# talmolab/VNL-Brax-Imitation

Measured on AMD Instinct MI355X. Metric: env-steps/sec (whole node), rodent imitation, num_envs=4096/GPU, higher is better.
Workload: dtype f32; 1 GPU; rodent imitation rollout, single groom clip, 4096 envs/GPU: intention-policy forward (HIP) -> RodentTracking.step (5 substeps, CG 6/6) -> auto-reset on -> Transition logging (unroll 20, the 20 steps replayed as one captured hipGraph); envs_per_gpu=4096, clips=1, parallelism=env-sharded x1, no data-path collective

## Files before the change

__graft_entry__.py:

```python
from __future__ import annotations

import os
import sys

ROOT = os.path.dirname(os.path.abspath(__file__))
if ROOT not in sys.path:
    sys.path.insert(0, ROOT)


def build() -> None:
    import vnl_brax_imitation_amd
    from vnl_brax_imitation_amd.csrc import build as hip_build

    from concurrent.futures import ThreadPoolExecutor

    with ThreadPoolExecutor(9) as pool:
        futs = {v: pool.submit(hip_build.build, variant=v)
                for v in ("product", "spill", "noblk", "nospec", "tail", "plain", "vmemplain", "ldsplain", "sgprplain")}
        paths = {v: f.result() for v, f in futs.items()}
    path = paths["product"]
    assert all(os.path.exists(p_) for p_ in paths.values()), paths
    from oracle import oracle as _oracle

    _oracle.build()
    from vnl_brax_imitation_amd import _lib

    _lib.load_library(path)
    print(f"[build] {path} ok; oracle ok")


def smoke() -> None:
    import numpy as np
    import torch

    sys.path.insert(0, os.path.join(ROOT, "tests"))
    import helpers as H
    from vnl_brax_imitation_amd.envs.rodent import RodentTracking

    assert torch.cuda.is_available(), "smoke() needs a HIP device"
    B = 256
    env = RodentTracking(H.reference_clip(), num_envs=B, device="cuda:0", **H.env_kwargs())
    rng = np.random.default_rng(0)
    sf = rng.integers(0, 235, B).astype(np.int32)
    noise = (1e-3 * rng.standard_normal((B, 74))).astype(np.float32)
    st = env.reset(start_frame=torch.from_numpy(sf), noise=torch.from_numpy(noise))
    act = np.clip(0.3 * rng.standard_normal((B, 30)), -1, 1).astype(np.float32)
    o = H.make_oracle(env, "f64")
    ost = o.env_reset(sf, noise)
    e_reset = H.scaled_err(st.pipeline_state.qacc_warmstart.cpu().numpy(), ost["qacc_warmstart"])
    e_obs = H.scaled_err(st.obs.cpu().numpy(), ost["obs"])
    import parity as P
# ... 33 lines not shown
```

vnl-brax-imitation_amd/csrc/build.py:

```python
from __future__ import annotations

import os
import subprocess
import sys

HERE = os.path.dirname(os.path.abspath(__file__))
SOURCES = ["vnl_lib.hip", "vnl_policy.hip", "vnl_ppo.hip", "vnl_domain.hip"]
DEPS = SOURCES + ["vnl_env_kernels.h", "vnl_body.h", "vnl_types.h", "vnl_philox.h", "vnl_policy_train.h", "../../include/vnl.h"]
OUT = os.path.join(HERE, "libvnl.so")

VARIANTS = {
    "product": ("libvnl.so", ["-DVNL_KERNEL_ATTR=__attribute__((amdgpu_waves_per_eu(2,2)))"]),
    "prof": ("libvnl_prof.so", ["-DVNL_PROFILE", "-DVNL_KERNEL_ATTR=__attribute__((amdgpu_waves_per_eu(2,2)))"]),
    "knobs": ("libvnl_knobs.so", ["-DVNL_STAGE_KNOBS", "-DVNL_KERNEL_ATTR=__attribute__((amdgpu_waves_per_eu(2,2)))"]),
    "spill": ("libvnl_spill.so", ["-DVNL_KERNEL_ATTR=__attribute__((amdgpu_waves_per_eu(4,4)))"]),
    "noblk": ("libvnl_noblk.so", ["-DVNL_NO_BLK", "-DVNL_KERNEL_ATTR=__attribute__((amdgpu_waves_per_eu(2,2)))"]),
    "tail": ("libvnl_tail.so", ["-DVNL_SOLVER_TAIL", "-DVNL_KERNEL_ATTR=__attribute__((amdgpu_waves_per_eu(2,2)))"]),
    "plain": ("libvnl_plain.so", ["-DVNL_SOLVER_PLAIN", "-DVNL_KERNEL_ATTR=__attribute__((amdgpu_waves_per_eu(2,2)))"]),
    "vmemplain": ("libvnl_vmemplain.so", ["-DVNL_VMEM_PLAIN", "-DVNL_KERNEL_ATTR=__attribute__((amdgpu_waves_per_eu(2,2)))"]),
    "ldsplain": ("libvnl_ldsplain.so", ["-DVNL_LDS_PLAIN", "-DVNL_KERNEL_ATTR=__attribute__((amdgpu_waves_per_eu(2,2)))"]),
    "sgprplain": ("libvnl_sgprplain.so", ["-DVNL_SGPR_PLAIN", "-DVNL_KERNEL_ATTR=__attribute__((amdgpu_waves_per_eu(2,2)))"]),
    "nospec": ("libvnl_nospec.so", ["-DVNL_NO_SPEC", "-DVNL_KERNEL_ATTR=__attribute__((amdgpu_waves_per_eu(2,2)))"]),
}
ENV_KERNELS = ("vnl_step_kernel", "vnl_reset_kernel", "vnl_reset_done_kernel")


def resource_usage(stderr_text: str) -> dict:
    out, name = {}, None
    for line in stderr_text.splitlines():
        if "Function Name:" in line:
            name = line.split("Function Name:")[1].split()[0]
            out[name] = {}
        elif name and "remark:" in line:
            body = line.split("remark:")[1].split("[-Rpass")[0].strip()
            key, _, val = body.rpartition(":")
            try:
                out[name][key.strip()] = int(val.strip())
            except ValueError:
                pass
    return out


def build(force: bool = False, verbose: bool = False, profile: bool = False, knobs: bool = False,
          variant: str | None = None) -> str:
    variant = variant or ("prof" if profile else ("knobs" if knobs else "product"))
    fname, defs = VARIANTS[variant]
    out = os.path.join(HERE, fname)
    deps = [os.path.join(HERE, d) for d in DEPS] + [os.path.abspath(__file__)]
    newest = max(os.path.getmtime(d) for d in deps)
    if not force and os.path.exists(out) and os.path.getmtime(out) >= newest:
        return out
    hipcc = os.environ.get("HIPCC", "/opt/rocm/bin/hipcc")
    objdir = os.path.join(HERE, "_obj", variant)
    os.makedirs(objdir, exist_ok=True)
# ... 68 lines not shown
```

vnl-brax-imitation_amd/csrc/vnl_body.h:

```cpp
#pragma once
#include <math.h>
#ifdef VNL_FORKJOIN_DEFINED
#include <assert.h>
#endif

#include "vnl_types.h"

#ifndef VNL_HD
#define VNL_HD __device__ __forceinline__
#endif
#include "vnl_philox.h"

#ifndef VNL_FORKJOIN_DEFINED
#define VNL_LANES 64
#define VNL_ROWS_PER_LANE 8
#define VNL_ROWS_SMALL 5
#define VNL_CHAIN_WIDTH 8
#define VNL_ROWSETS_1 1
#define VNL_ROWSETS_2 2
#define VNL_FOR(i, n) for (int i = (int)lane; i < (n); i += VNL_LANES)
#define VNL_SERIAL if (lane == 0)
#define VNL_SYNC() __builtin_amdgcn_fence(__ATOMIC_ACQ_REL, "wavefront")
#define VNL_SYNC_GLOBAL()                                     \
  do {                                                        \
    __builtin_amdgcn_fence(__ATOMIC_ACQ_REL, "wavefront");    \
    asm volatile("s_waitcnt vmcnt(0)" ::: "memory");          \
    __builtin_amdgcn_fence(__ATOMIC_ACQ_REL, "wavefront");    \
  } while (0)
#define VNL_LDS_DECL(name) extern __shared__ __align__(16) vreal name[]
VNL_HD float vnl_wave_sum(float x) {
#define VNL_DPP_STEP(ctrl) x += __builtin_bit_cast(float, __builtin_amdgcn_update_dpp(0, __builtin_bit_cast(int, x), ctrl, 0xf, 0xf, true))
  VNL_DPP_STEP(0xB1);
  VNL_DPP_STEP(0x4E);
  VNL_DPP_STEP(0x141);
  VNL_DPP_STEP(0x140);
#undef VNL_DPP_STEP
  x += __builtin_bit_cast(float, __builtin_amdgcn_update_dpp(0, __builtin_bit_cast(int, x), 0x142, 0xa, 0xf, false));
  x += __builtin_bit_cast(float, __builtin_amdgcn_update_dpp(0, __builtin_bit_cast(int, x), 0x143, 0xc, 0xf, false));
  return __builtin_bit_cast(float, __builtin_amdgcn_readlane(__builtin_bit_cast(int, x), 63));
}
VNL_HD float vnl_wave_sum16(float x) {
#define VNL_DPP_STEP(ctrl) x += __builtin_bit_cast(float, __builtin_amdgcn_update_dpp(0, __builtin_bit_cast(int, x), ctrl, 0xf, 0xf, true))
  VNL_DPP_STEP(0xB1);
  VNL_DPP_STEP(0x4E);
  VNL_DPP_STEP(0x141);
  VNL_DPP_STEP(0x140);
#undef VNL_DPP_STEP
  return __builtin_bit_cast(float, __builtin_amdgcn_readlane(__builtin_bit_cast(int, x), 0));
}
VNL_HD bool vnl_wave_any(bool x) { return __ballot(x) != 0ull; }
VNL_HD float vnl_wave_scan(float x) {
#define VNL_DPP_SCAN(ctrl, rmask) \
  x += __builtin_bit_cast(float, __builtin_amdgcn_update_dpp(0, __builtin_bit_cast(int, x), ctrl, rmask, 0xf, false))
  VNL_DPP_SCAN(0x111, 0xf);
  VNL_DPP_SCAN(0x112, 0xf);
  VNL_DPP_SCAN(0x114, 0xf);
  VNL_DPP_SCAN(0x118, 0xf);
  VNL_DPP_SCAN(0x142, 0xa);
  VNL_DPP_SCAN(0x143, 0xc);
#undef VNL_DPP_SCAN
  return x;
}
#define VNL_SCAN_ADD(x, run) (x = vnl_wave_scan(x))
#define VNL_WAVE_ITEMS(n) VNL_LANES
#define VNL_PAD_ITEMS(n) (((n) + VNL_LANES - 1) / VNL_LANES * VNL_LANES)
#define VNL_SCAN_ADD_C(x, run, carry) \
  (x = vnl_wave_scan(x) + carry, carry = __builtin_bit_cast(float, __builtin_amdgcn_readlane(__builtin_bit_cast(int, x), 63)))
#define VNL_PERLANE(T, name) T name
#define VNL_AT(name, j) name
#define VNL_GETF(name, a) __builtin_bit_cast(float, __builtin_amdgcn_readlane(__builtin_bit_cast(int, name), a))
#define VNL_GETI(name, a) __builtin_amdgcn_readlane(name, a)
#define VNL_ROWGETI(name, q, l) __builtin_amdgcn_readlane(name[q], l)
#define VNL_ROWGETF(expr, q, l) __builtin_bit_cast(float, __builtin_amdgcn_readlane(__builtin_bit_cast(int, expr), l))
VNL_HD float vnl_seg_sum(float x, unsigned cont, int steps) {
#define VNL_DPP_SEG(ctrl, bit)                                                                                          \
  do {                                                                                                                  \
    const float t_ = __builtin_bit_cast(float, __builtin_amdgcn_update_dpp(0, __builtin_bit_cast(int, x), ctrl, 0xf, 0xf, true)); \
    x += (cont & (bit)) ? t_ : 0.0f;                                                                                     \
  } while (0)
  if (steps > 0) VNL_DPP_SEG(0x101, 1u);
  if (steps > 1) VNL_DPP_SEG(0x102, 2u);
  if (steps > 2) VNL_DPP_SEG(0x104, 4u);
  if (steps > 3) VNL_DPP_SEG(0x108, 8u);
#undef VNL_DPP_SEG
  return x;
}
#define VNL_SEG_SUM(part, dsc, steps) (part = vnl_seg_sum(part, (dsc) >> 28, steps))
#define VNL_WAVE_FENCE() __builtin_amdgcn_fence(__ATOMIC_ACQ_REL, "wavefront")
#define VNL_LINE_HEADERS(out, base, stride)                                                       \
  do {                                                                                            \
    int hv_ = (int)(base)[((int)lane < VNL_FAC_LINES ? (int)lane : VNL_FAC_LINES - 1) * (stride)]; \
    _Pragma("unroll") for (int k_ = 0; k_ < VNL_FAC_LINES; k_++) out[k_] = __builtin_amdgcn_readlane(hv_, k_); \
  } while (0)
#define VNL_COUNT(pred) __popcll(__ballot(pred))
#define VNL_RANK(pred, run, rank)                                                   \
  do {                                                                              \
    const unsigned long long b_ = __ballot(pred);                                   \
    rank = run + (int)__popcll(b_ & ((1ull << (threadIdx.x & 63)) - 1ull));         \
    run += (int)__popcll(b_);                                                       \
  } while (0)
#define VNL_UNIFORM_I(x) __builtin_amdgcn_readfirstlane(x)
VNL_HD float vnl_recip(float x) {
  float r = __builtin_amdgcn_rcpf(x);
  return r * (2.0f - x * r);
}
#endif

#ifndef VNL_FORKJOIN_DEFINED
VNL_HD void vnl_count_add(uint32_t* p) { atomicAdd(p, 1u); }
VNL_HD int vnl_cdf_cell(const uint32_t* cdf, int ncell, uint32_t x, unsigned lane) {
  int lo = 0, len = ncell - 1;
  while (len > VNL_LANES) {
    const int stride = (len + VNL_LANES - 1) / VNL_LANES, end = lo + len;
    const int p = lo + ((int)lane + 1) * stride - 1;
    const bool le = p < end && cdf[p] <= x;
    const int k = (int)__popcll(__ballot(le));
    lo = lo + k * stride < end ? lo + k * stride : end;
    len = end - lo < stride - 1 ? end - lo : stride - 1;
  }
  const bool le = (int)lane < len && cdf[lo + (int)lane] <= x;
  return lo + (int)__popcll(__ballot(le));
}
#else
VNL_HD void vnl_count_add(uint32_t* p) { *p += 1u; }
VNL_HD int vnl_cdf_cell(const uint32_t* cdf, int ncell, uint32_t x, unsigned) {
  int lo = 0, hi = ncell - 1;
  while (lo < hi) {
    const int mid = (lo + hi) >> 1;
    if (cdf[mid] <= x) lo = mid + 1; else hi = mid;
  }
  return lo;
}
#endif

#ifdef VNL_PROFILE
#define VNL_NPROF 40
__device__ unsigned long long g_vnl_prof[VNL_NPROF];
#define VNL_PROF(i)                                                                             \
// ... 429 lines not shown
  }

  VNL_HD void body_inertias(bool with_com) const {
    V3 O = ref_point();
    V3 csum = v3(vreal(0.), vreal(0.), vreal(0.));
    VNL_FOR(b, MI(nbody)) {
      int o = LO(P) + 10 * b;
      if (b == 0) {
        for (int k = 0; k < 10; k++) s[o + k] = vreal(0.);
        continue;
      }
      const int ob = m.body_out[b];
      M3 R = qmat(gquat4(ob));
      vreal mass = par_row<P_MASS>()[b];
      V3 xip = gpos3(ob) + mmul(R, t3(par_row<P_IPOS>(), b));
      csum = csum + xip * mass;
      V3 r = xip - O;
      const vreal* I6 = par_row<P_INERTIA6>() + 6 * b;
      vreal Ib[9] = {I6[0], I6[3], I6[4], I6[3], I6[1], I6[5], I6[4], I6[5], I6[2]};
      vreal T[9];
      for (int i = 0; i < 3; i++)
        for (int k = 0; k < 3; k++)
          T[3 * i + k] = R.a[3 * i] * Ib[k] + R.a[3 * i + 1] * Ib[3 + k] + R.a[3 * i + 2] * Ib[6 + k];
      vreal rr = dot(r, r);
      s[o + 0] = T[0] * R.a[0] + T[1] * R.a[1] + T[2] * R.a[2] + mass * (rr - r.x * r.x);
      s[o + 1] = T[3] * R.a[3] + T[4] * R.a[4] + T[5] * R.a[5] + mass * (rr - r.y * r.y);
      s[o + 2] = T[6] * R.a[6] + T[7] * R.a[7] + T[8] * R.a[8] + mass * (rr - r.z * r.z);
      s[o + 3] = T[0] * R.a[3] + T[1] * R.a[4] + T[2] * R.a[5] - mass * r.x * r.y;
      s[o + 4] = T[0] * R.a[6] + T[1] * R.a[7] + T[2] * R.a[8] - mass * r.x * r.z;
      s[o + 5] = T[3] * R.a[6] + T[4] * R.a[7] + T[5] * R.a[8] - mass * r.y * r.z;
      s[o + 6] = r.x * mass, s[o + 7] = r.y * mass, s[o + 8] = r.z * mass, s[o + 9] = mass;
    }
    if (with_com) {
      vreal cx = vnl_wave_sum(csum.x), cy = vnl_wave_sum(csum.y), cz = vnl_wave_sum(csum.z);
      VNL_SERIAL { st3(LO(com), v3(cx * total_mass_inv(), cy * total_mass_inv(), cz * total_mass_inv())); }
    }
    VNL_SYNC();
  }

  VNL_HD void tree_accumulate(int base, int width) const {
    VNL_FOR(k, width) {
      vreal carry = vreal(0.);
      int b = MI(nbody) - 1;
      constexpr int G = 8;
      for (; b >= 1 && (b & (G - 1)) != G - 1; b--) {
        const int o = base + width * b + k;
        const vreal v = s[o] + carry;
        const int p = parent_of(b);
        if (carry != vreal(0.)) s[o] = v;
        if (p == b - 1) {
          carry = v;
        } else {
          carry = vreal(0.);
          if (p > 0) s[base + width * p + k] += v;
        }
      }
      for (; b >= G - 1; b -= G) {
        const int b0 = b - (G - 1);
        const int o = base + width * b0 + k;
        unsigned pw[G / 4];
#pragma unroll
        for (int j = 0; j < G / 4; j++) pw[j] = (unsigned)VNL_UNIFORM_I((int)((const unsigned*)(s + LO(tab_body)))[(b0 >> 2) + j]);
        vreal x[G], x0[G];
#pragma unroll
        for (int j = 0; j < G; j++) x0[j] = x[j] = s[o + width * j];
#pragma unroll
        for (int j = G - 1; j >= 0; j--) {
// ... 910 lines not shown
    int X0 = LO(P) + 10 * MI(nbody);
    dof_prefix(LO(qvel), LO(LD));
    const int cv = cvel_at();
    VNL_FOR(b, MI(nbody)) st6(cv + 6 * b, path_sum(LO(LD), m.body_pathseg + 8 * b));
    VNL_SYNC();
    VNL_PROF(2);
    int ca = X0;
    const int QB = LO(LD) + 6 * (MI(nv) + 1);
    S6 run = S6{v3(0, 0, 0), v3(0, 0, 0)}, carry = run;
    VNL_FOR(b, VNL_PAD_ITEMS(MI(nbody))) {
      S6 acc = S6{v3(0, 0, 0), v3(0, 0, 0)};
      if (b > 0 && b < MI(nbody)) {
        S6 vel = ld6(cv + 6 * parent_of(b));
        int jn = m.body_jntnum[b], ja = m.body_jntadr[b];
        for (int k = 0; k < jn; k++) {
          int j = ja + k, da = m.jnt_dofadr[j];
          if (m.jnt_type[j] == VNL_JNT_FREE) {
            for (int t = 0; t < 3; t++) vel = vel + ld6(LO(cdof) + 6 * (da + t)) * s[LO(qvel) + da + t];
            S6 vel0 = vel;
            for (int t = 3; t < 6; t++) {
              S6 c = ld6(LO(cdof) + 6 * (da + t));
              vreal qd = s[LO(qvel) + da + t];
              acc = acc + mcross(vel0, c) * qd;
              vel = vel + c * qd;
            }
          } else {
            S6 c = ld6(LO(cdof) + 6 * da);
            vreal qd = s[LO(qvel) + da];
            acc = acc + mcross(vel, c) * qd;
            vel = vel + c * qd;
          }
        }
      }
      VNL_SCAN_ADD_C(acc.a.x, run.a.x, carry.a.x), VNL_SCAN_ADD_C(acc.a.y, run.a.y, carry.a.y);
      VNL_SCAN_ADD_C(acc.a.z, run.a.z, carry.a.z), VNL_SCAN_ADD_C(acc.l.x, run.l.x, carry.l.x);
      VNL_SCAN_ADD_C(acc.l.y, run.l.y, carry.l.y), VNL_SCAN_ADD_C(acc.l.z, run.l.z, carry.l.z);
      if (b < MI(nbody)) st6(QB + 6 * (b + 1), acc);
      if (b == 0) st6(QB, S6{v3(0, 0, 0), v3(0, 0, 0)});
    }
    VNL_SYNC();
    VNL_FOR(b, MI(nbody)) st6(ca + 6 * b, path_sum(QB, m.body_pathseg + 8 * b + 4));
    VNL_SYNC();
    VNL_PROF(3);
    VNL_FOR(b, MI(nbody)) {
      if (b == 0) {
        st6(ca, S6{v3(0, 0, 0), v3(0, 0, 0)});
        continue;
      }
      S6 vel = ld6(cv + 6 * b), acc = ld6(ca + 6 * b);
      acc.l = acc.l + v3(-m.gx, -m.gy, -m.gz);
      st6(ca + 6 * b, inert_mul(LO(P) + 10 * b, acc) + mcross_force(vel, inert_mul(LO(P) + 10 * b, vel)));
    }
    VNL_SYNC();
    tree_accumulate(ca, 6);
    VNL_FOR(d, MI(nv))
      s[LO(smooth) + d] = -par<P_DAMP>(d) * s[LO(qvel) + d] - dot(ld6(LO(cdof) + 6 * d), ld6(ca + 6 * m.dof_body[d]));
    VNL_SYNC();
    VNL_PROF(4);
    return cv;
  }

  VNL_HD void smooth_forces() const {
    VNL_FOR(j, MI(njnt)) {
#ifdef VNL_VMEM_PLAIN
      if (m.jnt_type[j] == VNL_JNT_HINGE) {
        vreal k = m.jnt_stiffness[j];
        if (k != vreal(0.)) s[LO(smooth) + m.jnt_dofadr[j]] -= k * (s[LO(qpos) + m.jnt_qposadr[j]] - m.jnt_springref[j]);
      }
#else
// ... 148 lines not shown
      VNL_SERIAL { ((int*)(s + LO(act_list)))[(MI(ncon) + 3) / 4] = na; }
    }
    VNL_FOR(r, MI(nefc)) s[LO(jv) + r] = vreal(0.);
    {
      unsigned short* lv = live_rows();
      int nl = 0;
      VNL_FOR(r, VNL_PAD_ITEMS(MI(nefc))) {
        const bool on = r < MI(nefc) && s[LO(efc_D) + (r < MI(nefc) ? r : 0)] != vreal(0.);
        int pos;
        VNL_RANK(on, nl, pos);
        if (on && pos < VNL_LIVE_MAX) lv[pos] = (unsigned short)r;
      }
      VNL_SERIAL { ((int*)(s + LO(act_list)))[(MI(ncon) + 3) / 4 + 1] = nl; }
    }
    VNL_SYNC();
    if (trace) {
      VNL_SERIAL {
        VNL_ROLLED
        for (int w = 0; w < 16; w++) {
          int bits = 0;
          VNL_ROLLED
          for (int b = 0; b < 32; b++) {
            const int r = 32 * w + b;
            if (r < MI(nefc) && s[LO(efc_D) + r] != vreal(0.)) bits |= 1 << b;
          }
          trace[VNL_TRACE_ROWS + w] = bits;
        }
      }
    }
  }

  VNL_HD void dof_prefix(int vec, int Q) const {
    S6 run = S6{v3(0, 0, 0), v3(0, 0, 0)}, carry = run;
    VNL_FOR(d, VNL_PAD_ITEMS(MI(nv))) {
      S6 x = S6{v3(0, 0, 0), v3(0, 0, 0)};
      if (d < MI(nv)) x = ld6(LO(cdof) + 6 * d) * s[vec + d];
      VNL_SCAN_ADD_C(x.a.x, run.a.x, carry.a.x), VNL_SCAN_ADD_C(x.a.y, run.a.y, carry.a.y);
      VNL_SCAN_ADD_C(x.a.z, run.a.z, carry.a.z), VNL_SCAN_ADD_C(x.l.x, run.l.x, carry.l.x);
      VNL_SCAN_ADD_C(x.l.y, run.l.y, carry.l.y), VNL_SCAN_ADD_C(x.l.z, run.l.z, carry.l.z);
      if (d < MI(nv)) st6(Q + 6 * (d + 1), x);
      if (d == 0) st6(Q, S6{v3(0, 0, 0), v3(0, 0, 0)});
    }
    VNL_SYNC();
  }
  template <class RUN>
  VNL_HD S6 path_sum_runs(int Q, RUN run) const {
    S6 acc = S6{v3(0, 0, 0), v3(0, 0, 0)};
#pragma unroll
    for (int k = 0; k < 4; k++) {
      if (k >= MI(path_runs)) break;
      const int sg = run(k), b = sg & 0xff, e = sg >> 8;
      S6 qe = ld6(Q + 6 * e), qb = ld6(Q + 6 * b);
      acc = S6{acc.a + (qe.a - qb.a), acc.l + (qe.l - qb.l)};
    }
    return acc;
  }
  VNL_HD S6 path_sum(int Q, const int* seg) const { return path_sum_runs(Q, [&](int k) { return seg[k]; }); }
  VNL_HD S6 path_sum_con(int Q, int c) const { return path_sum_runs(Q, [&](int k) { return con_path_run(c, k); }); }

  VNL_HD void jac_mul(int vec, int out, bool accumulate) const {
    V3 n = v3(m.pnx, m.pny, m.pnz);
    for_live_rows([&](int r) {
      if (r < MI(nlimit)) {
        vreal v = copysign(vreal(1.), s[LO(efc_D) + r]) * s[vec + lim_dof_of(r)];
        s[out + r] = accumulate ? s[out + r] + v : v;
      }
    });
    const int Q = LO(P) + 3 * MI(nefc);
    dof_prefix(vec, Q);
    const unsigned char* act = (const unsigned char*)(s + LO(act_list));
    int na = ((const int*)(s + LO(act_list)))[(MI(ncon) + 3) / 4];
    VNL_FOR(j, na) {
      int c = act[j], g = con_geom_of(c), r0 = MI(nlimit) + 4 * c;
      S6 vel = path_sum_con(Q, c);
      vreal mu = con_mu_of(g);
// ... 17 lines not shown
  }

  VNL_HD vreal constraint_force() const {
    V3 n = v3(m.pnx, m.pny, m.pnz);
    int Wc = LO(P) + 3 * MI(nefc);
    vreal cost = vreal(0.);
    for_live_rows([&](int r) {
      if (r < MI(nlimit)) {
        vreal x = s[LO(Jaref) + r];
        cost += x < vreal(0.) ? fabs(s[LO(efc_D) + r]) * x * x : vreal(0.);
      }
    });
    {
      S6 run = S6{v3(0, 0, 0), v3(0, 0, 0)};
      VNL_FOR(k, VNL_WAVE_ITEMS(MI(ncon))) {
        S6 w = S6{v3(0, 0, 0), v3(0, 0, 0)};
        if (k < MI(ncon)) {
          const int c = con_ordered(k);
          int r0 = MI(nlimit) + 4 * c;
          vreal D = s[LO(efc_D) + r0];
          if (D != vreal(0.)) {
            int g = con_geom_of(c);
            vreal mu = con_mu_of(g), f[4];
            for (int q = 0; q < 4; q++) {
              vreal x = s[LO(Jaref) + r0 + q];
              f[q] = x < vreal(0.) ? -D * x : vreal(0.);
              cost += x < vreal(0.) ? D * x * x : vreal(0.);
            }
            V3 rel = ld3(LO(con_r) + 3 * c), t1 = ld3(LO(con_t1) + 3 * g), t2 = cross(n, t1);
            V3 Fw = n * (f[0] + f[1] + f[2] + f[3]) + t1 * (mu * (f[0] - f[1])) + t2 * (mu * (f[2] - f[3]));
            w = S6{cross(rel, Fw), Fw};
          }
        }
        VNL_SCAN_ADD(w.a.x, run.a.x), VNL_SCAN_ADD(w.a.y, run.a.y), VNL_SCAN_ADD(w.a.z, run.a.z);
        VNL_SCAN_ADD(w.l.x, run.l.x), VNL_SCAN_ADD(w.l.y, run.l.y), VNL_SCAN_ADD(w.l.z, run.l.z);
        if (k < MI(ncon)) st6(Wc + 6 * (k + 1), w);
        if (k == 0) st6(Wc, S6{v3(0, 0, 0), v3(0, 0, 0)});
      }
      VNL_SYNC();
      VNL_FOR(d, MI(nv)) {
        const int pk = limrow_of(d), r = (pk & 0x3ff) - 1, c0 = (pk >> 10) & 0xff, c1 = (pk >> 18) & 0xff;
        S6 p1 = ld6(Wc + 6 * c1), p0 = ld6(Wc + 6 * c0);
        S6 w = S6{p1.a - p0.a, p1.l - p0.l};
        vreal q = dot(ld6(LO(cdof) + 6 * d), w);
        if (r >= 0) {
          vreal x = s[LO(Jaref) + r];
          q += x < vreal(0.) ? -s[LO(efc_D) + r] * x : vreal(0.);
        }
        s[LO(qfrc_c) + d] = q;
      }
      VNL_SYNC();
      return vreal(0.5) * vnl_wave_sum(cost);
    }
    return vreal(0.);
  }

  VNL_HD vreal vdot(int a, int b) const {
    vreal p = vreal(0.);
    VNL_FOR(d, MI(nv)) p += s[a + d] * s[b + d];
    return vnl_wave_sum(p);
  }

  struct LsPoint {
    vreal alpha, cost, d0, d1;
  };
  template <int RPL>
  struct LsRows {
    vreal ja[RPL], jv[RPL], a0[RPL], a1[RPL], a2[RPL];
// ... 9 lines not shown
      n += VNL_COUNT(live && R.ja[j] + alpha * R.jv[j] < vreal(0.));
    }
    return n;
  }
  template <int RPL>
  VNL_HD void ls_load(LsRows<RPL>& R, bool compact) const {
#pragma unroll
    for (int j = 0; j < RPL; j++) {
      int r = (int)lane + j * VNL_LANES;
      bool ok = r < MI(nefc);
      if (compact) {
        ok = r < num_live_rows();
        r = ok ? (int)live_rows()[r] : 0;
      }
      vreal D = ok ? fabs(s[LO(efc_D) + r]) : vreal(0.);
      vreal ja = ok ? s[LO(Jaref) + r] : vreal(0.), jv = ok ? s[LO(jv) + r] : vreal(0.);
      R.ja[j] = ja, R.jv[j] = jv;
      R.a0[j] = vreal(0.5) * ja * ja * D, R.a1[j] = jv * ja * D, R.a2[j] = vreal(0.5) * jv * jv * D;
    }
  }
  template <int N, int RPL>
  VNL_HD void ls_eval(const LsRows<RPL>& R, const vreal* alpha, vreal qg0, vreal qg1, vreal qg2, LsPoint* out, bool few = false) const {
    vreal q0[N], q1[N], q2[N];
    for (int i = 0; i < N; i++) q0[i] = vreal(0.), q1[i] = vreal(0.), q2[i] = vreal(0.);
#pragma unroll
    for (int j = 0; j < RPL; j++) {
      for (int i = 0; i < N; i++) {
        bool act = R.ja[j] + alpha[i] * R.jv[j] < vreal(0.);
        q0[i] += act ? R.a0[j] : vreal(0.), q1[i] += act ? R.a1[j] : vreal(0.), q2[i] += act ? R.a2[j] : vreal(0.);
      }
    }
    if (few) {
      for (int i = 0; i < N; i++) q0[i] = vnl_wave_sum16(q0[i]), q1[i] = vnl_wave_sum16(q1[i]), q2[i] = vnl_wave_sum16(q2[i]);
    } else {
      for (int i = 0; i < N; i++) q0[i] = vnl_wave_sum(q0[i]), q1[i] = vnl_wave_sum(q1[i]), q2[i] = vnl_wave_sum(q2[i]);
    }
    for (int i = 0; i < N; i++) {
      vreal t0 = qg0 + q0[i], t1 = qg1 + q1[i], t2 = qg2 + q2[i];
      vreal a = alpha[i];
      out[i].alpha = a;
      out[i].cost = a * a * t2 + a * t1 + t0;
      out[i].d0 = vreal(2.) * a * t2 + t1;
      out[i].d1 = vreal(2.) * t2 + (t2 == vreal(0.) ? VNL_MINVAL : vreal(0.));
    }
  }

  template <int RPL, bool COMPACT = false>
  VNL_HD vreal line_search(vreal gauss, vreal qg1, vreal qg2, vreal gtol, int* tr ) const {
      LsPoint p0, lo, hi;
      LsRows<RPL> rows;
      ls_load(rows, COMPACT);
      const bool few = COMPACT && RPL == 1 && VNL_LANES >= 16 && num_live_rows() <= 16;
      vreal a1[1] = {vreal(0.)};
      ls_eval<1>(rows, a1, gauss, qg1, qg2, &p0, few);
      if (tr) {
        const int n0 = ls_count_active(rows, a1[0], COMPACT);
        VNL_SERIAL { tr[4] = n0, tr[24] = __builtin_bit_cast(int, (float)a1[0]); }
      }
      a1[0] = p0.alpha - p0.d0 / p0.d1;
      ls_eval<1>(rows, a1, gauss, qg1, qg2, &lo, few);
      if (tr) {
        const int n1 = ls_count_active(rows, a1[0], COMPACT);
        VNL_SERIAL { tr[5] = n1, tr[25] = __builtin_bit_cast(int, (float)a1[0]); }
      }
      if (tr) {
        const int first_lo = lo.d0 < p0.d0;
        VNL_SERIAL { tr[2] |= first_lo << 24; }
      }
// ... 138 lines not shown
    vreal gauss = use_warm ? vreal(0.5) * gw : vreal(0.);
    vreal cost = fresh().constraint_force() + gauss;
    vreal prev_cost = INFINITY;
    vreal gg = vreal(0.), ss = vreal(0.), gp = vreal(0.);
    VNL_FOR(d, nv) {
      vreal g = s[LO(Ma) + d] - s[LO(smooth) + d] - s[LO(qfrc_c) + d];
      s[LO(grad) + d] = g, s[LO(Mgrad) + d] = g;
      gg += g * g;
    }
    gg = vnl_wave_sum(gg);
    VNL_SYNC();
    const bool newton = MI(solver_newton) != 0;
    if (newton) fresh().newton_solve(LO(Mgrad));
    else fresh().solve_inplace(LO(Mgrad));
#ifdef VNL_LDS_PLAIN
    const bool qg_carried = false;
#else
    const bool qg_carried = !newton;
#endif
    vreal qg1c = vreal(0.), qg2c = vreal(0.);
    VNL_FOR(d, nv) {
      const vreal mg = s[LO(Mgrad) + d], gr = s[LO(grad) + d];
      s[LO(search) + d] = -mg;
      s[LO(mv) + d] = -gr;
      ss += mg * mg, gp += gr * mg;
      if (qg_carried) {
        vreal sd = -mg, md = -gr;
        VNL_OPAQUE(sd);
        VNL_OPAQUE(md);
        qg1c += sd * s[LO(Ma) + d] - sd * s[LO(smooth) + d];
        qg2c += sd * md;
      }
    }
    ss = vnl_wave_sum(ss), gp = vnl_wave_sum(gp);
    if (qg_carried) qg1c = vnl_wave_sum(qg1c), qg2c = vreal(0.5) * vnl_wave_sum(qg2c);
    VNL_SYNC();
    if (newton) fresh().newton_mass_mul(LO(search), LO(mv));
    VNL_PROF(15);

    for (int it = 0; it < MI(iterations); it++) {
      vreal improvement = (prev_cost - cost) / m.scale;
      vreal gradient = sqrt(gg) / m.scale;
      if (improvement < m.tolerance || gradient < m.tolerance) break;
      vreal smag = sqrt(ss) * m.scale;
      vreal gtol = m.tolerance * m.ls_tolerance * smag;
      VNL_PROF(16);
      fresh().jac_mul(LO(search), LO(jv), false);
      VNL_PROF(17);
      vreal qg1 = qg1c, qg2 = qg2c;
      if (!qg_carried) {
        qg1 = vreal(0.), qg2 = vreal(0.);
        VNL_FOR(d, nv) {
          vreal sd = s[LO(search) + d];
          qg1 += sd * s[LO(Ma) + d] - sd * s[LO(smooth) + d];
          qg2 += sd * s[LO(mv) + d];
        }
        qg1 = vnl_wave_sum(qg1), qg2 = vreal(0.5) * vnl_wave_sum(qg2);
      }
      VNL_PROF(18);
      int* tr = (trace && it < VNL_TRACE_ITERS) ? trace + 8 + VNL_TRACE_REC * it : nullptr;
      if (trace) {
        VNL_SYNC();
        VNL_SERIAL { trace[1] = it + 1; }
      }
      const int nlive = num_live_rows();
      vreal alpha = (nlive <= (VNL_LANES < VNL_LIVE_MAX ? VNL_LANES : VNL_LIVE_MAX))
                        ? fresh().template line_search<1, true>(gauss, qg1, qg2, gtol, tr)
                        : (nlive <= (2 * VNL_LANES < VNL_LIVE_MAX ? 2 * VNL_LANES : VNL_LIVE_MAX))
                        ? fresh().template line_search<2, true>(gauss, qg1, qg2, gtol, tr)
                        : ((MI(nefc) <= 5 * VNL_LANES) ? fresh().template line_search<VNL_ROWS_SMALL>(gauss, qg1, qg2, gtol, tr)
                                                     : fresh().template line_search<VNL_ROWS_PER_LANE>(gauss, qg1, qg2, gtol, tr));
#ifdef VNL_LDS_PLAIN
      VNL_FOR(d, nv) {
        s[LO(qacc) + d] += alpha * s[LO(search) + d];
        s[LO(Ma) + d] += alpha * s[LO(mv) + d];
      }
#else
      vreal g = vreal(0.);
      VNL_FOR(d, nv) {
        vreal qa = s[LO(qacc) + d], ma = s[LO(Ma) + d];
        qa += alpha * s[LO(search) + d];
        ma += alpha * s[LO(mv) + d];
        VNL_OPAQUE(qa);
        VNL_OPAQUE(ma);
        s[LO(qacc) + d] = qa, s[LO(Ma) + d] = ma;
        g += (ma - s[LO(smooth) + d]) * (qa - s[LO(qacc_smooth) + d]);
      }
#endif
      VNL_PROF(19);
      for_live_rows([&](int r) { s[LO(Jaref) + r] += alpha * s[LO(jv) + r]; });
      VNL_SYNC();
      VNL_PROF(20);
#ifndef VNL_SOLVER_TAIL
      if (it + 1 >= MI(iterations) && !trace) {
        (void)fresh().constraint_force();
        VNL_PROF(22);
        break;
      }
#endif
#ifdef VNL_LDS_PLAIN
      vreal g = vreal(0.);
      VNL_FOR(d, nv) g += (s[LO(Ma) + d] - s[LO(smooth) + d]) * (s[LO(qacc) + d] - s[LO(qacc_smooth) + d]);
#endif
      g = vnl_wave_sum(g);
      VNL_PROF(21);
      vreal ncost = fresh().constraint_force() + vreal(0.5) * g;
      VNL_PROF(22);
      prev_cost = cost, cost = ncost, gauss = vreal(0.5) * g;
      vreal d1 = vreal(0.);
      gg = vreal(0.);
      VNL_FOR(d, nv) {
        vreal gn = s[LO(Ma) + d] - s[LO(smooth) + d] - s[LO(qfrc_c) + d];
        d1 += gn * s[LO(Mgrad) + d];
        s[LO(grad) + d] = gn, s[LO(tmp) + d] = gn;
        gg += gn * gn;
      }
      d1 = vnl_wave_sum(d1), gg = vnl_wave_sum(gg);
      VNL_SYNC();
      VNL_PROF(23);
      if (newton) fresh().newton_solve(LO(tmp));
      else fresh().solve_inplace(LO(tmp));
      VNL_PROF(24);
      vreal d2 = vdot(LO(grad), LO(tmp));
      vreal beta = fmax(vreal(0.), (d2 - d1) / fmax(VNL_MINVAL, gp));
      if (newton) beta = vreal(0.);
      gp = d2;
      ss = vreal(0.);
#ifdef VNL_LDS_PLAIN
      VNL_FOR(d, nv) {
        vreal mg = s[LO(tmp) + d];
        s[LO(Mgrad) + d] = mg;
        const vreal sn = -mg + beta * s[LO(search) + d];
        s[LO(search) + d] = sn;
        s[LO(mv) + d] = -s[LO(grad) + d] + beta * s[LO(mv) + d];
        ss += sn * sn;
      }
#else
      qg1c = vreal(0.), qg2c = vreal(0.);
      VNL_FOR(d, nv) {
        vreal mg = s[LO(tmp) + d];
        s[LO(Mgrad) + d] = mg;
        vreal sn = -mg + beta * s[LO(search) + d];
        vreal mn = -s[LO(grad) + d] + beta * s[LO(mv) + d];
        VNL_OPAQUE(sn);
        VNL_OPAQUE(mn);
        s[LO(search) + d] = sn;
        s[LO(mv) + d] = mn;
        ss += sn * sn;
        if (qg_carried) {
          qg1c += sn * s[LO(Ma) + d] - sn * s[LO(smooth) + d];
          qg2c += sn * mn;
        }
      }
#endif
      ss = vnl_wave_sum(ss);
      if (qg_carried) qg1c = vnl_wave_sum(qg1c), qg2c = vreal(0.5) * vnl_wave_sum(qg2c);
      VNL_SYNC();
      if (newton) fresh().newton_mass_mul(LO(search), LO(mv));
      VNL_PROF(25);
    }
  }

  VNL_HD void forward(const vreal* gwarm) const {
#ifdef VNL_VMEM_PLAIN
    const vreal* warm = gwarm ? gwarm : s + LO(qacc);
    VNL_FOR(d, MI(nv)) s[LO(tmp) + d] = warm[d];
    VNL_SYNC();
    VNL_FOR(d, MI(nv)) s[LO(qacc) + d] = s[LO(tmp) + d];
    VNL_SYNC();
#else
    if (gwarm) {
      const auto* gw = VNL_GLOBAL_PTR(vreal, gwarm);
      VNL_FOR(d, MI(nv)) s[LO(qacc) + d] = gw[d];
      VNL_SYNC();
    }
#endif
#ifdef VNL_STAGE_KNOBS
    for (int rep = 0; rep < m.dbg_count; rep++) {
      if (m.dbg_stage == 1) {
        kinematics();
        body_inertias(false);
        mass_matrix(vreal(0.));
        factor();
        invert_factor();
      } else if (m.dbg_stage == 2) {
        kinematics();
      } else if (m.dbg_stage == 3) {
        kinematics();
        body_inertias(false);
// ... 177 lines not shown
        Q4 r = qmul(ld4(LO(qpos) + qa + 3), Q4{cs, ax.x * sn, ax.y * sn, ax.z * sn});
        vreal n2 = sqrt(r.w * r.w + r.x * r.x + r.y * r.y + r.z * r.z);
        vreal inv = n2 > vreal(0.) ? vreal(1.) / n2 : vreal(1.);
        s[LO(qpos) + qa + 3] = r.w * inv, s[LO(qpos) + qa + 4] = r.x * inv, s[LO(qpos) + qa + 5] = r.y * inv,
                        s[LO(qpos) + qa + 6] = r.z * inv;
      } else {
        s[LO(qpos) + qa] += m.dt * s[LO(qvel) + da];
      }
    }
    VNL_SYNC();
    VNL_PROF(28);
  }

  VNL_HD static int clampi(int v, int lo, int hi) { return v < lo ? lo : (v > hi ? hi : v); }
  VNL_HD static vreal nan0(vreal x) {
    if (x != x) return vreal(0.);
    if (x > vreal(3.4028235e38)) return vreal(3.4028235e38);
    if (x < -vreal(3.4028235e38)) return -vreal(3.4028235e38);
    return x;
  }

  VNL_HD vreal termination(int clip, int frame, const vreal* qpos, const vreal* xpos) const {
    int f = clampi(frame, 0, ev.T - 1), nj = MI(nq) - 7;
    const float* cj = ev.joints + ((size_t)clip * ev.T + f) * nj;
    const float* cb = ev.body_positions + ((size_t)clip * ev.T + f) * ev.nb * 3;
    vreal ej = vreal(0.), cx = vreal(0.), cy = vreal(0.), cz = vreal(0.);
    VNL_FOR(i, nj) ej += fabs(vreal(cj[i]) - qpos[7 + i]);
    VNL_FOR(k, ev.nb) {
      int bd = ev.body_idxs[k];
      cx += fabs(vreal(cb[3 * k]) - xpos[3 * bd]);
      cy += fabs(vreal(cb[3 * k + 1]) - xpos[3 * bd + 1]);
      cz += fabs(vreal(cb[3 * k + 2]) - xpos[3 * bd + 2]);
    }
    ej = vnl_wave_sum(ej), cx = vnl_wave_sum(cx), cy = vnl_wave_sum(cy), cz = vnl_wave_sum(cz);
    vreal eb = fmax(cx, fmax(cy, cz));
    if (ev.flags & VNL_ENV_TERM_MEAN) {
      eb = (cx + cy + cz) / vreal(3 * ev.nb);
      ej = ej / vreal(nj);
    }
    vreal err = vreal(0.5) * ev.body_err_mult * eb + vreal(0.5) * ej;
    return vreal(1.) - err * ev.inv_term_threshold;
  }

  VNL_HD void load_state() const {
    const vreal* gq = st.qpos + (size_t)e * MI(nq);
    const vreal* gv = st.qvel + (size_t)e * MI(nv);
    const vreal* ga = st.act + (size_t)e * MI(nu);
    VNL_FOR(i, MI(nq)) s[LO(qpos) + i] = gq[i];
    VNL_FOR(i, MI(nv)) s[LO(qvel) + i] = gv[i];
    VNL_FOR(i, MI(nu)) s[LO(act) + i] = ga[i];
    VNL_SYNC();
  }

  VNL_HD bool store_state() const {
    vreal* gq = st.qpos + (size_t)e * MI(nq);
    vreal* gv = st.qvel + (size_t)e * MI(nv);
    vreal* ga = st.act + (size_t)e * MI(nu);
    vreal* gw = st.warm + (size_t)e * MI(nv);
    const vreal* gf = gqfrc_act();
    const vreal* gx = gxpos();
    bool bad = false;
    VNL_FOR(i, MI(nq)) {
      vreal v = s[LO(qpos) + i];
      gq[i] = v, bad |= v != v;
    }
    VNL_FOR(i, MI(nv)) {
      vreal a = s[LO(qvel) + i], b = s[LO(qacc) + i], c = gf[i];
// ... 325 lines not shown
```

Baseline: 2.783 million env-steps/s.

## Batch wave reductions and scans into shared DPP row-broadcast inline asm

Replaces per-value wave sums and scans with batched versions. Each value gets its own within-row DPP reduction, then one inline-asm block performs the row_bcast15/31 cross-row joins for several values together, so the required s_nop hazard waits are shared instead of paid once per value. It also adds a tail path in dof_prefix that scans a short final chunk of up to 16 DOFs with a single row scan across lanes. The change aims to cut cross-lane latency in the solver, the CoM, the RNE scans and termination. In exchange it relies on hand-written DPP asm whose hazard handling must be correct, and it adds an xlaneplain build variant for A/B comparison.

Measured after the change: 2.909 million env-steps/s (median of 6 runs). +4.5%, better.

```diff
diff --git a/__graft_entry__.py b/__graft_entry__.py
--- a/__graft_entry__.py
+++ b/__graft_entry__.py
@@ -14,9 +14,10 @@
 
     from concurrent.futures import ThreadPoolExecutor
 
-    with ThreadPoolExecutor(9) as pool:
+    with ThreadPoolExecutor(10) as pool:
         futs = {v: pool.submit(hip_build.build, variant=v)
-                for v in ("product", "spill", "noblk", "nospec", "tail", "plain", "vmemplain", "ldsplain", "sgprplain")}
+                for v in ("product", "spill", "noblk", "nospec", "tail", "plain", "vmemplain", "ldsplain", "sgprplain",
+                          "xlaneplain")}
         paths = {v: f.result() for v, f in futs.items()}
     path = paths["product"]
     assert all(os.path.exists(p_) for p_ in paths.values()), paths
diff --git a/vnl-brax-imitation_amd/csrc/build.py b/vnl-brax-imitation_amd/csrc/build.py
--- a/vnl-brax-imitation_amd/csrc/build.py
+++ b/vnl-brax-imitation_amd/csrc/build.py
@@ -20,6 +20,7 @@
     "vmemplain": ("libvnl_vmemplain.so", ["-DVNL_VMEM_PLAIN", "-DVNL_KERNEL_ATTR=__attribute__((amdgpu_waves_per_eu(2,2)))"]),
     "ldsplain": ("libvnl_ldsplain.so", ["-DVNL_LDS_PLAIN", "-DVNL_KERNEL_ATTR=__attribute__((amdgpu_waves_per_eu(2,2)))"]),
     "sgprplain": ("libvnl_sgprplain.so", ["-DVNL_SGPR_PLAIN", "-DVNL_KERNEL_ATTR=__attribute__((amdgpu_waves_per_eu(2,2)))"]),
+    "xlaneplain": ("libvnl_xlaneplain.so", ["-DVNL_XLANE_PLAIN", "-DVNL_KERNEL_ATTR=__attribute__((amdgpu_waves_per_eu(2,2)))"]),
     "nospec": ("libvnl_nospec.so", ["-DVNL_NO_SPEC", "-DVNL_KERNEL_ATTR=__attribute__((amdgpu_waves_per_eu(2,2)))"]),
 }
 ENV_KERNELS = ("vnl_step_kernel", "vnl_reset_kernel", "vnl_reset_done_kernel")
diff --git a/vnl-brax-imitation_amd/csrc/vnl_body.h b/vnl-brax-imitation_amd/csrc/vnl_body.h
--- a/vnl-brax-imitation_amd/csrc/vnl_body.h
+++ b/vnl-brax-imitation_amd/csrc/vnl_body.h
@@ -28,6 +28,71 @@
     __builtin_amdgcn_fence(__ATOMIC_ACQ_REL, "wavefront");    \
   } while (0)
 #define VNL_LDS_DECL(name) extern __shared__ __align__(16) vreal name[]
+#if defined(__HIP_DEVICE_COMPILE__) && !defined(VNL_XLANE_PLAIN)
+#define VNL_XLANE 1
+#define VNL_B15_(n) "v_add_f32_dpp %" #n ", %" #n ", %" #n " row_bcast:15 row_mask:0xa bank_mask:0xf\n\t"
+#define VNL_B31_(n) "v_add_f32_dpp %" #n ", %" #n ", %" #n " row_bcast:31 row_mask:0xc bank_mask:0xf\n\t"
+VNL_HD void vnl_rows_join(float& a) { asm("s_nop 1\n\t" VNL_B15_(0) "s_nop 1\n\t" VNL_B31_(0) : "+v"(a)); }
+VNL_HD void vnl_rows_join(float& a, float& b) {
+  asm("s_nop 1\n\t" VNL_B15_(0) VNL_B15_(1) "s_nop 0\n\t" VNL_B31_(0) VNL_B31_(1) : "+v"(a), "+v"(b));
+}
+VNL_HD void vnl_rows_join(float& a, float& b, float& c) {
+  asm("s_nop 1\n\t" VNL_B15_(0) VNL_B15_(1) VNL_B15_(2) VNL_B31_(0) VNL_B31_(1) VNL_B31_(2) : "+v"(a), "+v"(b), "+v"(c));
+}
+VNL_HD void vnl_rows_join(float& a, float& b, float& c, float& d) {
+  asm("s_nop 1\n\t" VNL_B15_(0) VNL_B15_(1) VNL_B15_(2) VNL_B15_(3) VNL_B31_(0) VNL_B31_(1) VNL_B31_(2) VNL_B31_(3)
+      : "+v"(a), "+v"(b), "+v"(c), "+v"(d));
+}
+VNL_HD void vnl_rows_join(float& a, float& b, float& c, float& d, float& e, float& f) {
+  asm("s_nop 1\n\t" VNL_B15_(0) VNL_B15_(1) VNL_B15_(2) VNL_B15_(3) VNL_B15_(4) VNL_B15_(5)
+      VNL_B31_(0) VNL_B31_(1) VNL_B31_(2) VNL_B31_(3) VNL_B31_(4) VNL_B31_(5)
+      : "+v"(a), "+v"(b), "+v"(c), "+v"(d), "+v"(e), "+v"(f));
+}
+VNL_HD void vnl_rows_join(float& a, float& b, float& c, float& d, float& e, float& f, float& g, float& h, float& i) {
+  asm("s_nop 1\n\t" VNL_B15_(0) VNL_B15_(1) VNL_B15_(2) VNL_B15_(3) VNL_B15_(4) VNL_B15_(5) VNL_B15_(6) VNL_B15_(7) VNL_B15_(8)
+      VNL_B31_(0) VNL_B31_(1) VNL_B31_(2) VNL_B31_(3) VNL_B31_(4) VNL_B31_(5) VNL_B31_(6) VNL_B31_(7) VNL_B31_(8)
+      : "+v"(a), "+v"(b), "+v"(c), "+v"(d), "+v"(e), "+v"(f), "+v"(g), "+v"(h), "+v"(i));
+}
+#undef VNL_B15_
+#undef VNL_B31_
+VNL_HD float vnl_row_sum(float x) {
+#define VNL_DPP_STEP(ctrl) x += __builtin_bit_cast(float, __builtin_amdgcn_update_dpp(0, __builtin_bit_cast(int, x), ctrl, 0xf, 0xf, true))
+  VNL_DPP_STEP(0xB1);
+  VNL_DPP_STEP(0x4E);
+  VNL_DPP_STEP(0x141);
+  VNL_DPP_STEP(0x140);
+#undef VNL_DPP_STEP
+  return x;
+}
+VNL_HD float vnl_last_lane(float x) { return __builtin_bit_cast(float, __builtin_amdgcn_readlane(__builtin_bit_cast(int, x), 63)); }
+VNL_HD float vnl_wave_sum(float x) {
+  x = vnl_row_sum(x);
+  vnl_rows_join(x);
+  return vnl_last_lane(x);
+}
+VNL_HD void vnl_wave_sums(float& a, float& b) {
+  a = vnl_row_sum(a), b = vnl_row_sum(b);
+  vnl_rows_join(a, b);
+  a = vnl_last_lane(a), b = vnl_last_lane(b);
+}
+VNL_HD void vnl_wave_sums(float& a, float& b, float& c) {
+  a = vnl_row_sum(a), b = vnl_row_sum(b), c = vnl_row_sum(c);
+  vnl_rows_join(a, b, c);
+  a = vnl_last_lane(a), b = vnl_last_lane(b), c = vnl_last_lane(c);
+}
+VNL_HD void vnl_wave_sums(float& a, float& b, float& c, float& d) {
+  a = vnl_row_sum(a), b = vnl_row_sum(b), c = vnl_row_sum(c), d = vnl_row_sum(d);
+  vnl_rows_join(a, b, c, d);
+  a = vnl_last_lane(a), b = vnl_last_lane(b), c = vnl_last_lane(c), d = vnl_last_lane(d);
+}
+VNL_HD void vnl_wave_sums(float& a, float& b, float& c, float& d, float& e, float& f, float& g, float& h, float& i) {
+  a = vnl_row_sum(a), b = vnl_row_sum(b), c = vnl_row_sum(c), d = vnl_row_sum(d), e = vnl_row_sum(e);
+  f = vnl_row_sum(f), g = vnl_row_sum(g), h = vnl_row_sum(h), i = vnl_row_sum(i);
+  vnl_rows_join(a, b, c, d, e, f, g, h, i);
+  a = vnl_last_lane(a), b = vnl_last_lane(b), c = vnl_last_lane(c), d = vnl_last_lane(d), e = vnl_last_lane(e);
+  f = vnl_last_lane(f), g = vnl_last_lane(g), h = vnl_last_lane(h), i = vnl_last_lane(i);
+}
+#else
 VNL_HD float vnl_wave_sum(float x) {
 #define VNL_DPP_STEP(ctrl) x += __builtin_bit_cast(float, __builtin_amdgcn_update_dpp(0, __builtin_bit_cast(int, x), ctrl, 0xf, 0xf, true))
   VNL_DPP_STEP(0xB1);
@@ -39,6 +104,7 @@
   x += __builtin_bit_cast(float, __builtin_amdgcn_update_dpp(0, __builtin_bit_cast(int, x), 0x143, 0xc, 0xf, false));
   return __builtin_bit_cast(float, __builtin_amdgcn_readlane(__builtin_bit_cast(int, x), 63));
 }
+#endif
 VNL_HD float vnl_wave_sum16(float x) {
 #define VNL_DPP_STEP(ctrl) x += __builtin_bit_cast(float, __builtin_amdgcn_update_dpp(0, __builtin_bit_cast(int, x), ctrl, 0xf, 0xf, true))
   VNL_DPP_STEP(0xB1);
@@ -49,6 +115,27 @@
   return __builtin_bit_cast(float, __builtin_amdgcn_readlane(__builtin_bit_cast(int, x), 0));
 }
 VNL_HD bool vnl_wave_any(bool x) { return __ballot(x) != 0ull; }
+#ifdef VNL_XLANE
+VNL_HD float vnl_row_scan(float x) {
+#define VNL_DPP_SCAN(ctrl) \
+  x += __builtin_bit_cast(float, __builtin_amdgcn_update_dpp(0, __builtin_bit_cast(int, x), ctrl, 0xf, 0xf, false))
+  VNL_DPP_SCAN(0x111);
+  VNL_DPP_SCAN(0x112);
+  VNL_DPP_SCAN(0x114);
+  VNL_DPP_SCAN(0x118);
+#undef VNL_DPP_SCAN
+  return x;
+}
+VNL_HD float vnl_wave_scan(float x) {
+  x = vnl_row_scan(x);
+  vnl_rows_join(x);
+  return x;
+}
+VNL_HD void vnl_wave_scan6(float& a, float& b, float& c, float& d, float& e, float& f) {
+  a = vnl_row_scan(a), b = vnl_row_scan(b), c = vnl_row_scan(c), d = vnl_row_scan(d), e = vnl_row_scan(e), f = vnl_row_scan(f);
+  vnl_rows_join(a, b, c, d, e, f);
+}
+#else
 VNL_HD float vnl_wave_scan(float x) {
 #define VNL_DPP_SCAN(ctrl, rmask) \
   x += __builtin_bit_cast(float, __builtin_amdgcn_update_dpp(0, __builtin_bit_cast(int, x), ctrl, rmask, 0xf, false))
@@ -61,6 +148,7 @@
 #undef VNL_DPP_SCAN
   return x;
 }
+#endif
 #define VNL_SCAN_ADD(x, run) (x = vnl_wave_scan(x))
 #define VNL_WAVE_ITEMS(n) VNL_LANES
 #define VNL_PAD_ITEMS(n) (((n) + VNL_LANES - 1) / VNL_LANES * VNL_LANES)
@@ -104,6 +192,34 @@
   float r = __builtin_amdgcn_rcpf(x);
   return r * (2.0f - x * r);
 }
+#endif
+
+#ifdef VNL_XLANE
+#define VNL_WAVE_SUMS(...) vnl_wave_sums(__VA_ARGS__)
+#define VNL_SCAN6(v, run) vnl_wave_scan6(v.a.x, v.a.y, v.a.z, v.l.x, v.l.y, v.l.z)
+#define VNL_SCAN6_C(v, run, cy)                                                          \
+  do {                                                                                      \
+    vnl_wave_scan6(v.a.x, v.a.y, v.a.z, v.l.x, v.l.y, v.l.z);                               \
+    v.a = v.a + cy.a, v.l = v.l + cy.l;                                               \
+    cy.a = v3(vnl_last_lane(v.a.x), vnl_last_lane(v.a.y), vnl_last_lane(v.a.z));         \
+    cy.l = v3(vnl_last_lane(v.l.x), vnl_last_lane(v.l.y), vnl_last_lane(v.l.z));         \
+  } while (0)
+#else
+#define VNL_SUM1_(x) (x = vnl_wave_sum(x))
+#define VNL_SUMS_2_(a, b) (VNL_SUM1_(a), VNL_SUM1_(b))
+#define VNL_SUMS_3_(a, b, c) (VNL_SUM1_(a), VNL_SUM1_(b), VNL_SUM1_(c))
+#define VNL_SUMS_4_(a, b, c, d) (VNL_SUM1_(a), VNL_SUM1_(b), VNL_SUM1_(c), VNL_SUM1_(d))
+#define VNL_SUMS_9_(a, b, c, d, e, f, g, h, i) (VNL_SUMS_4_(a, b, c, d), VNL_SUMS_4_(e, f, g, h), VNL_SUM1_(i))
+#define VNL_SUMS_PICK_(a, b, c, d, e, f, g, h, i, name, ...) name
+#define VNL_WAVE_SUMS(...) \
+  VNL_SUMS_PICK_(__VA_ARGS__, VNL_SUMS_9_, x, x, x, x, VNL_SUMS_4_, VNL_SUMS_3_, VNL_SUMS_2_, x)(__VA_ARGS__)
+#define VNL_SCAN6(v, run)                                                                                    \
+  (VNL_SCAN_ADD(v.a.x, run.a.x), VNL_SCAN_ADD(v.a.y, run.a.y), VNL_SCAN_ADD(v.a.z, run.a.z),                 \
+   VNL_SCAN_ADD(v.l.x, run.l.x), VNL_SCAN_ADD(v.l.y, run.l.y), VNL_SCAN_ADD(v.l.z, run.l.z))
+#define VNL_SCAN6_C(v, run, cy)                                                                           \
+  (VNL_SCAN_ADD_C(v.a.x, run.a.x, cy.a.x), VNL_SCAN_ADD_C(v.a.y, run.a.y, cy.a.y),                     \
+   VNL_SCAN_ADD_C(v.a.z, run.a.z, cy.a.z), VNL_SCAN_ADD_C(v.l.x, run.l.x, cy.l.x),                     \
+   VNL_SCAN_ADD_C(v.l.y, run.l.y, cy.l.y), VNL_SCAN_ADD_C(v.l.z, run.l.z, cy.l.z))
 #endif
 
 #ifndef VNL_FORKJOIN_DEFINED
@@ -599,7 +715,8 @@
       s[o + 6] = r.x * mass, s[o + 7] = r.y * mass, s[o + 8] = r.z * mass, s[o + 9] = mass;
     }
     if (with_com) {
-      vreal cx = vnl_wave_sum(csum.x), cy = vnl_wave_sum(csum.y), cz = vnl_wave_sum(csum.z);
+      vreal cx = csum.x, cy = csum.y, cz = csum.z;
+      VNL_WAVE_SUMS(cx, cy, cz);
       VNL_SERIAL { st3(LO(com), v3(cx * total_mass_inv(), cy * total_mass_inv(), cz * total_mass_inv())); }
     }
     VNL_SYNC();
@@ -1576,9 +1693,7 @@
           }
         }
       }
-      VNL_SCAN_ADD_C(acc.a.x, run.a.x, carry.a.x), VNL_SCAN_ADD_C(acc.a.y, run.a.y, carry.a.y);
-      VNL_SCAN_ADD_C(acc.a.z, run.a.z, carry.a.z), VNL_SCAN_ADD_C(acc.l.x, run.l.x, carry.l.x);
-      VNL_SCAN_ADD_C(acc.l.y, run.l.y, carry.l.y), VNL_SCAN_ADD_C(acc.l.z, run.l.z, carry.l.z);
+      VNL_SCAN6_C(acc, run, carry);
       if (b < MI(nbody)) st6(QB + 6 * (b + 1), acc);
       if (b == 0) st6(QB, S6{v3(0, 0, 0), v3(0, 0, 0)});
     }
@@ -1793,15 +1908,46 @@
 
   VNL_HD void dof_prefix(int vec, int Q) const {
     S6 run = S6{v3(0, 0, 0), v3(0, 0, 0)}, carry = run;
-    VNL_FOR(d, VNL_PAD_ITEMS(MI(nv))) {
+#ifdef VNL_XLANE
+    const int last = (MI(nv) - 1) / VNL_LANES * VNL_LANES, rem = MI(nv) - last;
+    const bool tail = last > 0 && rem <= 16;
+    const int full = tail ? last : VNL_PAD_ITEMS(MI(nv));
+#else
+    const int full = VNL_PAD_ITEMS(MI(nv));
+#endif
+    VNL_FOR(d, full) {
       S6 x = S6{v3(0, 0, 0), v3(0, 0, 0)};
       if (d < MI(nv)) x = ld6(LO(cdof) + 6 * d) * s[vec + d];
-      VNL_SCAN_ADD_C(x.a.x, run.a.x, carry.a.x), VNL_SCAN_ADD_C(x.a.y, run.a.y, carry.a.y);
-      VNL_SCAN_ADD_C(x.a.z, run.a.z, carry.a.z), VNL_SCAN_ADD_C(x.l.x, run.l.x, carry.l.x);
-      VNL_SCAN_ADD_C(x.l.y, run.l.y, carry.l.y), VNL_SCAN_ADD_C(x.l.z, run.l.z, carry.l.z);
+#ifdef VNL_XLANE
+      VNL_OPAQUE(x.a.x);
+      VNL_OPAQUE(x.a.y);
+      VNL_OPAQUE(x.a.z);
+      VNL_OPAQUE(x.l.x);
+      VNL_OPAQUE(x.l.y);
+      VNL_OPAQUE(x.l.z);
+#endif
+      VNL_SCAN6_C(x, run, carry);
       if (d < MI(nv)) st6(Q + 6 * (d + 1), x);
       if (d == 0) st6(Q, S6{v3(0, 0, 0), v3(0, 0, 0)});
     }
+#ifdef VNL_XLANE
+    if (tail) {
+      const int t = (int)lane & 15, k = (int)lane >> 4, d = last + t;
+#pragma unroll
+      for (int h = 0; h < 2; h++) {
+        const int c = 4 * h + k;
+        const bool on = t < rem && c < 6;
+        vreal x = vreal(0.);
+        if (on) x = s[LO(cdof) + 6 * d + c] * s[vec + d];
+        VNL_OPAQUE(x);
+        x = vnl_row_scan(x);
+        const vreal cr = h == 0 ? (k == 0 ? carry.a.x : k == 1 ? carry.a.y : k == 2 ? carry.a.z : carry.l.x)
+                                : (k == 0 ? carry.l.y : carry.l.z);
+        x = x + cr;
+        if (on) s[Q + 6 * (d + 1) + c] = x;
+      }
+    }
+#endif
     VNL_SYNC();
   }
   template <class RUN>
@@ -1885,8 +2031,7 @@
             w = S6{cross(rel, Fw), Fw};
           }
         }
-        VNL_SCAN_ADD(w.a.x, run.a.x), VNL_SCAN_ADD(w.a.y, run.a.y), VNL_SCAN_ADD(w.a.z, run.a.z);
-        VNL_SCAN_ADD(w.l.x, run.l.x), VNL_SCAN_ADD(w.l.y, run.l.y), VNL_SCAN_ADD(w.l.z, run.l.z);
+        VNL_SCAN6(w, run);
         if (k < MI(ncon)) st6(Wc + 6 * (k + 1), w);
         if (k == 0) st6(Wc, S6{v3(0, 0, 0), v3(0, 0, 0)});
       }
@@ -1962,8 +2107,10 @@
     }
     if (few) {
       for (int i = 0; i < N; i++) q0[i] = vnl_wave_sum16(q0[i]), q1[i] = vnl_wave_sum16(q1[i]), q2[i] = vnl_wave_sum16(q2[i]);
+    } else if constexpr (N == 3) {
+      VNL_WAVE_SUMS(q0[0], q1[0], q2[0], q0[1], q1[1], q2[1], q0[2], q1[2], q2[2]);
     } else {
-      for (int i = 0; i < N; i++) q0[i] = vnl_wave_sum(q0[i]), q1[i] = vnl_wave_sum(q1[i]), q2[i] = vnl_wave_sum(q2[i]);
+      for (int i = 0; i < N; i++) VNL_WAVE_SUMS(q0[i], q1[i], q2[i]);
     }
     for (int i = 0; i < N; i++) {
       vreal t0 = qg0 + q0[i], t1 = qg1 + q1[i], t2 = qg2 + q2[i];
@@ -2168,8 +2315,12 @@
         qg2c += sd * md;
       }
     }
-    ss = vnl_wave_sum(ss), gp = vnl_wave_sum(gp);
-    if (qg_carried) qg1c = vnl_wave_sum(qg1c), qg2c = vreal(0.5) * vnl_wave_sum(qg2c);
+    if (qg_carried) {
+      VNL_WAVE_SUMS(ss, gp, qg1c, qg2c);
+      qg2c = vreal(0.5) * qg2c;
+    } else {
+      VNL_WAVE_SUMS(ss, gp);
+    }
     VNL_SYNC();
     if (newton) fresh().newton_mass_mul(LO(search), LO(mv));
     VNL_PROF(15);
@@ -2191,7 +2342,8 @@
           qg1 += sd * s[LO(Ma) + d] - sd * s[LO(smooth) + d];
           qg2 += sd * s[LO(mv) + d];
         }
-        qg1 = vnl_wave_sum(qg1), qg2 = vreal(0.5) * vnl_wave_sum(qg2);
+        VNL_WAVE_SUMS(qg1, qg2);
+        qg2 = vreal(0.5) * qg2;
       }
       VNL_PROF(18);
       int* tr = (trace && it < VNL_TRACE_ITERS) ? trace + 8 + VNL_TRACE_REC * it : nullptr;
@@ -2251,7 +2403,7 @@
         s[LO(grad) + d] = gn, s[LO(tmp) + d] = gn;
         gg += gn * gn;
       }
-      d1 = vnl_wave_sum(d1), gg = vnl_wave_sum(gg);
+      VNL_WAVE_SUMS(d1, gg);
       VNL_SYNC();
       VNL_PROF(23);
       if (newton) fresh().newton_solve(LO(tmp));
@@ -2289,8 +2441,12 @@
         }
       }
 #endif
-      ss = vnl_wave_sum(ss);
-      if (qg_carried) qg1c = vnl_wave_sum(qg1c), qg2c = vreal(0.5) * vnl_wave_sum(qg2c);
+      if (qg_carried) {
+        VNL_WAVE_SUMS(ss, qg1c, qg2c);
+        qg2c = vreal(0.5) * qg2c;
+      } else {
+        ss = vnl_wave_sum(ss);
+      }
       VNL_SYNC();
       if (newton) fresh().newton_mass_mul(LO(search), LO(mv));
       VNL_PROF(25);
@@ -2534,7 +2690,7 @@
       cy += fabs(vreal(cb[3 * k + 1]) - xpos[3 * bd + 1]);
       cz += fabs(vreal(cb[3 * k + 2]) - xpos[3 * bd + 2]);
     }
-    ej = vnl_wave_sum(ej), cx = vnl_wave_sum(cx), cy = vnl_wave_sum(cy), cz = vnl_wave_sum(cz);
+    VNL_WAVE_SUMS(ej, cx, cy, cz);
     vreal eb = fmax(cx, fmax(cy, cz));
     if (ev.flags & VNL_ENV_TERM_MEAN) {
       eb = (cx + cy + cz) / vreal(3 * ev.nb);
```
